# dselivanov/rsparse

Hardware: AMD Instinct MI355X
Metric: als_iterations_per_sec (higher is better)
Workload: dtype f32 (Gram products of rows > 512 / <= 32 non-zeros as 2 x fp16 / 3 x bf16 split terms of the fp32 operands, fp32 accumulate; everything else fp32); 1 GPU; WRMF implicit ALS, CG(3), synthetic 10000000x1000000, 500155883 nnz, rank 128, lambda 0.1; survey_config=3, feedback=implicit, n_items=1000000, nnz=500155883, rank=128, solver=conjugate_gradient, cg_steps=3, parallelism=rows sharded x1, factors replicated

## Files before the change

rsparse_amd/csrc/wrmf_cg_mf.hip:

```cpp
#include <cstdio>
#include <utility>

#pragma clang diagnostic ignored "-Winline-asm"

#include "wrmf_internal.h"
#include "wrmf_device.h"

namespace rsparse_hip {
namespace {
using namespace dev;
constexpr int MF_A0 = 0;
#define MF_TOP "a255"
}
}

#include "wrmf_mf.h"

namespace rsparse_hip {
namespace {

__device__ __forceinline__ void cgm_operands_hi(const float (&x)[16], f16x8& h0, f16x8& h1) {
  float b0[8], b1[8];
#pragma unroll
  for (int e = 0; e < 8; e++) {
// ... 3 lines not shown
  }
  unsigned hh0[4], hh1[4];
#pragma unroll
  for (int q = 0; q < 4; q++) {
    const f32x2 v0 = {b0[2 * q], b0[2 * q + 1]}, v1 = {b1[2 * q], b1[2 * q + 1]};
    hh0[q] = __builtin_bit_cast(unsigned, __builtin_convertvector(v0, f16x2));
    hh1[q] = __builtin_bit_cast(unsigned, __builtin_convertvector(v1, f16x2));
  }
  h0 = pack_f16x8(hh0[0], hh0[1], hh0[2], hh0[3]);
  h1 = pack_f16x8(hh1[0], hh1[1], hh1[2], hh1[3]);
}

struct CgmOps {
  f16x8 ah[4], al[4], mh[4];
};
struct CgmProd {
  int T, kind, K, I;
};
constexpr CgmProd cgm_prod(int idx) {
  if (idx < 16) return {mf_tid(idx % 4, 0), idx / 4, 0, idx % 4};
  idx -= 16;
  if (idx < 12) return {mf_tid(1 + idx % 3, 1), idx / 3, 1, 1 + idx % 3};
  idx -= 12;
  const int w = idx % 3, K = w == 2 ? 3 : 2, I = w == 0 ? 2 : 3;
  return {mf_tid(I, K), idx / 3, K, I};
}
template <int T>
__device__ __forceinline__ void cgm_mma16(const f16x8& a, const f16x8& b) {
  asm volatile("v_mfma_f32_32x32x16_f16 a[%c2:%c3], %0, %1, a[%c2:%c3]" ::"v"(a), "v"(b), "i"(MF_A0 + 16 * T), "i"(MF_A0 + 16 * T + 15));
}

template <int NOPS>
struct CgmWave {
  union {
    float ring[3][2048];
    float T[32 * 36];
  };
  int midx[3][64];
  float mval[3][64];
  float gval[3][64];
  unsigned long long maddr[3][64];
  float vec[128];
  float x0[128];
  float rhs[128];
  double loss;
};
template <int NOPS>
struct CgmSmem {
  float4 G[10][64][4];
  CgmWave<NOPS> w[4];
};

template <class RD, class GV, class WV>
__device__ __forceinline__ void cgm_matvec(RD&& rd, GV&& gtile, WV& sw, const int n, const int hf, const int ln,
                                           const float (&pr)[4], float (&out)[4]) {
  wave_sync();
  if (hf == 0) {
#pragma unroll
    for (int I = 0; I < 4; I++) sw.vec[32 * I + n] = pr[I];
  }
  wave_sync();
  float dsum[4] = {0.f, 0.f, 0.f, 0.f};
  static_for<4>([&](auto kt) {
    constexpr int K = decltype(kt)::value;
    float pc[16];
#pragma unroll
    for (int q = 0; q < 4; q++) {
      const float4 t = *reinterpret_cast<const float4*>(&sw.vec[32 * K + 8 * q + 4 * hf]);
      pc[4 * q] = t.x; pc[4 * q + 1] = t.y; pc[4 * q + 2] = t.z; pc[4 * q + 3] = t.w;
    }
    float ts[16];
#pragma unroll
    for (int v = 0; v < 16; v++) ts[v] = 0.f;
    static_for<4 - K>([&](auto st) {
      constexpr int I = K + decltype(st)::value;
      constexpr int T = mf_tid(I, K);
      float g[16];
      gtile(std::integral_constant<int, T>{}, g);
      static_for<16>([&](auto vt) {
        constexpr int v = decltype(vt)::value;
        const float av = rd(std::integral_constant<int, T>{}, std::integral_constant<int, v>{}) + g[v];
        dsum[I] = fmaf(av, pc[v], dsum[I]);
        if constexpr (I > K) ts[v] = fmaf(av, pr[I], ts[v]);
      });
    });
    if constexpr (K < 3) {
      wave_sync();
#pragma unroll
      for (int v = 0; v < 16; v++) sw.T[(8 * (v >> 2) + 4 * hf + (v & 3)) * 36 + n] = ts[v];
      wave_sync();
      float s0 = 0.f, s1 = 0.f;
#pragma unroll
      for (int q = 0; q < 8; q++) {
        const float4 t = *reinterpret_cast<const float4*>(&sw.T[n * 36 + 4 * q]);
        s0 += t.x + t.z;
        s1 += t.y + t.w;
      }
      out[K] = s0 + s1;
    } else {
      out[K] = 0.f;
    }
  });
#pragma unroll
  for (int I = 0; I < 4; I++) {
    const unsigned du = __float_as_uint(dsum[I]);
    const auto sw2 = __builtin_amdgcn_permlane32_swap(du, du, false, false);
    out[I] += __uint_as_float(sw2[0]) + __uint_as_float(sw2[1]);
  }
}

__device__ __forceinline__ float cgm_dot(const float (&a)[4], const float (&b)[4], const int hf) {
  float s = (a[0] * b[0] + a[1] * b[1]) + (a[2] * b[2] + a[3] * b[3]);
  return wave_sum(hf == 0 ? s : 0.f);
}

template <bool SYM>
__device__ __forceinline__ void als_cg_mf_body(const AlsArgs& a, const int32_t* __restrict__ rows, const int n_rows, const int loss_slot0) {
  extern __shared__ __attribute__((aligned(16))) char cgm_smem[];
  CgmSmem<SYM ? 12 : 20>& sm = *reinterpret_cast<CgmSmem<SYM ? 12 : 20>*>(cgm_smem);
  const int lane = threadIdx.x & 63, wv = rfl((int)(threadIdx.x >> 6));
  CgmWave<SYM ? 12 : 20>& sw = sm.w[wv];
  constexpr int k = 128;
  {
    const bool below_one = a.ne_stats[2] != 0u;
    if (below_one == SYM) {
      if (lane == 0) a.loss_partials[loss_slot0 + 4 * blockIdx.x + wv] = 0.0;
      return;
    }
  }
  for (int e = threadIdx.x; e < 10 * 64 * 16; e += 256) {
    const int t = e / 1024, l = (e >> 4) & 63, v = e & 15;
    const int I = t >= 6 ? 3 : (t >= 3 ? 2 : (t >= 1 ? 1 : 0)), K = t - I * (I + 1) / 2;
    const int nn = l & 31, hh = l >> 5;
    reinterpret_cast<float*>(&sm.G[t][l][0])[v] = a.XtX[(size_t)(4 * (8 * (v >> 2) + 4 * hh + (v & 3)) + K) * k + 4 * nn + I];
  }
  if (lane == 0) sw.loss = 0.0;
  __syncthreads();

  auto uni = [](const float x) { return __int_as_float(__builtin_amdgcn_readfirstlane(__float_as_int(x))); };
  const int ex = rfl(fp16_scale_exp(fmaxf(__uint_as_float(a.ne_stats[0]), 1e-30f)));
  const float wmax = uni(fmaxf(__uint_as_float(a.ne_stats[1]) - 1.f, 1.f));
  const int ewb = rfl((int)((__float_as_uint(wmax) >> 23) & 0xffu));
  const float sx = uni(pow2(ex)), sw_ = uni(pow2(min(253, max(1, 253 - ewb))));
  const float un1 = uni(pow2(254 - ex));
  const float unw = uni(pow2(254 - min(253, max(1, 253 - ewb))));
  const int n_waves = 4 * gridDim.x;

  for (int it = 4 * blockIdx.x + wv; it < n_rows; it += n_waves) {
    const int row = rfl(rows[it]);
    const int p1 = rfl(a.col_ptrs[row]), p2 = rfl(a.col_ptrs[row + 1]);
    float* yrow = a.Y + (size_t)row * k;
    int ln = lane;
    asm volatile("" : "+v"(ln));
    sw.x0[ln] = yrow[ln];
    sw.x0[64 + ln] = yrow[64 + ln];
    MF_DRAIN();
    static_for<256>([&](auto rt) { mf_wr<decltype(rt)::value>(0.f); });
    f32x16 hi[4];
#pragma unroll
    for (int t = 0; t < 4; t++)
#pragma unroll
      for (int e = 0; e < 16; e++) hi[t][e] = 0.f;
    float u0 = 0.f, u1 = 0.f, csum = 0.f;
    float ua[4] = {0.f, 0.f, 0.f, 0.f};
    {
      const int nsteps = (p2 - p1 + 15) >> 4;
      const int hfl = ln >> 5;
      const unsigned long long xoff = reinterpret_cast<unsigned long long>(a.X) + 16ull * (unsigned)(ln & 31);
      const unsigned ring_lds = (unsigned)(uintptr_t)&sw.ring[0][0];
      const unsigned meta_lds = (unsigned)(uintptr_t)&sw.midx[0][0];
      auto request_meta = [&](const int c) __attribute__((always_inline)) {
        const int pos = min(p1 + 64 * c + ln, p2 - 1);
        const int* gi = a.row_idx + pos;
        const float* gv = a.vals + pos;
        const unsigned dst = meta_lds + 256u * (unsigned)(c % 3);
        unsigned keep;
        asm volatile(
            "s_mov_b32 %[k], m0\n\ts_mov_b32 m0, %[l]\n\ts_nop 0\n\t"
            "global_load_lds_dword %[gi], off\n\ts_add_u32 m0, m0, 0x300\n\ts_nop 0\n\t"
            "global_load_lds_dword %[gv], off\n\t"
            "s_mov_b32 m0, %[k]"
            : [k] "=&s"(keep)
            : [l] "s"(dst), [gi] "v"(gi), [gv] "v"(gv)
            : "memory", "scc");
      };
      auto request = [&](const int st, const int slot) __attribute__((always_inline)) {
        const uint4* ap = reinterpret_cast<const uint4*>(&sw.maddr[(st >> 2) % 3][16 * (st & 3) + 8 * hfl]);
        const uint4 q0 = ap[0], q1 = ap[1], q2 = ap[2], q3 = ap[3];
        auto at = [&](const unsigned lo, const unsigned hi2) { return xoff + (((unsigned long long)hi2 << 32) | lo); };
        const unsigned long long g0 = at(q0.x, q0.y), g1 = at(q0.z, q0.w), g2 = at(q1.x, q1.y), g3 = at(q1.z, q1.w);
        const unsigned long long g4 = at(q2.x, q2.y), g5 = at(q2.z, q2.w), g6 = at(q3.x, q3.y), g7 = at(q3.z, q3.w);
        const unsigned dst = ring_lds + 8192u * (unsigned)slot + 4096u;
        unsigned keep;
        asm volatile(
            "s_mov_b32 %[k], m0\n\ts_mov_b32 m0, %[l]\n\ts_nop 0\n\t"
            "global_load_lds_dwordx4 %[g0], off offset:-4096\n\t"
            "global_load_lds_dwordx4 %[g1], off offset:-3072\n\t"
            "global_load_lds_dwordx4 %[g2], off offset:-2048\n\t"
            "global_load_lds_dwordx4 %[g3], off offset:-1024\n\t"
            "global_load_lds_dwordx4 %[g4], off\n\t"
            "global_load_lds_dwordx4 %[g5], off offset:1024\n\t"
            "global_load_lds_dwordx4 %[g6], off offset:2048\n\t"
            "global_load_lds_dwordx4 %[g7], off offset:3072\n\t"
            "s_mov_b32 m0, %[k]"
            : [k] "=&s"(keep)
            : [l] "s"(dst), [g0] "v"(g0), [g1] "v"(g1), [g2] "v"(g2), [g3] "v"(g3), [g4] "v"(g4), [g5] "v"(g5), [g6] "v"(g6), [g7] "v"(g7)
            : "memory");
      };
      auto consume = [&](const int st, const float cvr, float (&xs0)[16], float (&xs1)[16]) __attribute__((always_inline)) {
        const int ccnt = min(16, p2 - (p1 + 16 * st));
        const bool inl = (ln & 15) < ccnt;
        const float cvj = inl ? cvr : 0.f;
        csum += ln < 16 ? cvj : 0.f;
        const float f2 = inl ? sx : 0.f;
        float f1;
        if constexpr (SYM) f1 = inl ? sx * __builtin_amdgcn_sqrtf(fmaxf(cvr - 1.f, 0.f) * sw_) : 0.f;
        else f1 = inl ? (cvr - 1.f) * sw_ : 0.f;
#pragma unroll
        for (int s2 = 0; s2 < 16; s2++) {
          const float cv = readlane_f(cvj, s2);
          u0 = fmaf(cv, xs0[s2], u0);
          u1 = fmaf(cv, xs1[s2], u1);
          const float s_m = readlane_f(f2, s2);
          xs0[s2] *= s_m;
          xs1[s2] *= s_m;
        }
        asm volatile("" : "+v"(u0), "+v"(u1));
        __builtin_amdgcn_sched_barrier(0);
        float (&xm0)[16] = xs0;
        float (&xm1)[16] = xs1;
        f16x8 ah[4], al[4], mh[4], bh[4], bl[4];
        auto m2_products = [&]() __attribute__((always_inline)) {
          static_for<4>([&](auto kt) {
            constexpr int K = decltype(kt)::value;
            static_for<4 - K>([&](auto st2) {
              constexpr int I = K + decltype(st2)::value;
              constexpr int T = mf_tid(I, K);
              if constexpr (T < 6) mf_mma16<10 + T>(mh[K], mh[I]);
// ... 86 lines not shown
        wc[0] = wc0;
        wg[0] = wg0;
        float4 va[2], vb[2];
        va[0] = va0;
        vb[0] = vb0;
        unsigned hm[4][4], hh[4][4], ll[4][4];
        static_for<4>([&](auto qt) {
          constexpr int q = decltype(qt)::value;
          if constexpr (q < 3) {
            va[(q + 1) & 1] = *reinterpret_cast<const float4*>(rs + (2 * q + 2) * 256);
            vb[(q + 1) & 1] = *reinterpret_cast<const float4*>(rs + (2 * q + 3) * 256);
            wc[(q + 1) & 1] = pc[q + 1];
            wg[(q + 1) & 1] = pg[q + 1];
          }
          const float c0 = wc[q & 1].x, c1 = wc[q & 1].y, g0 = wg[q & 1].x, g1 = wg[q & 1].y;
          const float4 xa = va[q & 1], xb = vb[q & 1];
          const float a0s[4] = {xa.x, xa.y, xa.z, xa.w}, a1s[4] = {xb.x, xb.y, xb.z, xb.w};
          static_for<4>([&](auto It) {
            constexpr int I = decltype(It)::value, u = 4 * q + I, m0 = (5 * u) / 2, m1 = (5 * (u + 1)) / 2;
            const float a0 = a0s[I], a1 = a1s[I];
            ua[I] = fmaf(c1, a1, fmaf(c0, a0, ua[I]));
            const float t0 = a0 * sx, t1 = a1 * sx;
            {
              const f32x2 tv = {t0, t1};
              hm[I][q] = __builtin_bit_cast(unsigned, __builtin_convertvector(tv, f16x2));
            }
            mm(std::integral_constant<int, m0>{}, P);
            __builtin_amdgcn_sched_barrier(0);
            {
              const f32x2 yv = {t0 * g0, t1 * g1};
              const unsigned hv = __builtin_bit_cast(unsigned, __builtin_convertvector(yv, f16x2));
              float r0, r1;
              asm("v_fma_mix_f32 %0, %1, %2, -%3 op_sel_hi:[0,0,1]" : "=v"(r0) : "v"(t0), "v"(g0), "v"(hv));
              asm("v_fma_mix_f32 %0, %1, %2, -%3 op_sel:[0,0,1] op_sel_hi:[0,0,1]" : "=v"(r1) : "v"(t1), "v"(g1), "v"(hv));
              const f32x2 rv = {r0, r1};
              hh[I][q] = hv;
              ll[I][q] = __builtin_bit_cast(unsigned, __builtin_convertvector(rv, f16x2));
            }
            mm(std::integral_constant<int, m0 + 1>{}, P);
            if constexpr (m1 - m0 == 3) {
              __builtin_amdgcn_sched_barrier(0);
              mm(std::integral_constant<int, m0 + 2>{}, P);
            }
            __builtin_amdgcn_sched_barrier(0);
          });
        });
#pragma unroll
        for (int I = 0; I < 4; I++) {
          N.mh[I] = pack_f16x8(hm[I][0], hm[I][1], hm[I][2], hm[I][3]);
          N.ah[I] = pack_f16x8(hh[I][0], hh[I][1], hh[I][2], hh[I][3]);
          N.al[I] = pack_f16x8(ll[I][0], ll[I][1], ll[I][2], ll[I][3]);
        }
      };
      wave_sync();
      request_meta(0);
      request_meta(1);
      asm volatile("s_waitcnt vmcnt(0)" ::: "memory");
      transform(0);
      request(0, 0);
      request(1, 1);
      const int tail_st = ((p2 - p1) & 15) ? nsteps - 1 : -1;
      int slot = 0;
      for (int c = 0; 4 * c < nsteps; c++) {
        bool done = false;
        static_for<4>([&](auto jt) {
          constexpr int j = decltype(jt)::value;
          const int st = 4 * c + j;
          if (done || st >= nsteps) { done = true; return; }
          const int slot2 = slot == 0 ? 2 : slot - 1;
          float4 fva, fvb;
          float2 fwc, fwg;
          auto first_reads = [&](const int sl, const int cs, const int jj) __attribute__((always_inline)) {
            const float* rs = &sw.ring[sl][0] + 128 * hfl + 4 * (ln & 31);
            fva = *reinterpret_cast<const float4*>(rs);
            fvb = *reinterpret_cast<const float4*>(rs + 256);
            fwc = *reinterpret_cast<const float2*>(&sw.mval[cs][16 * jj + 8 * hfl]);
            fwg = *reinterpret_cast<const float2*>(&sw.gval[cs][16 * jj + 8 * hfl]);
          };
          if constexpr (j == 1) transform(c + 1);
          const bool more = st + 2 < nsteps;
          if (more) {
            if constexpr (j == 1) asm volatile("s_waitcnt vmcnt(10)" ::: "memory");
            else asm volatile("s_waitcnt vmcnt(8)" ::: "memory");
            if constexpr (SYM) first_reads(slot, c % 3, j);
            request(st + 2, slot2);
            if constexpr (j == 0) request_meta(c + 2);
          } else {
            asm volatile("s_waitcnt vmcnt(0)" ::: "memory");
            if constexpr (SYM) {
              if (st == tail_st) zero_tail(slot, (p2 - p1) & 15);
              first_reads(slot, c % 3, j);
            }
          }
          if constexpr (SYM) {
            __builtin_amdgcn_sched_barrier(0);
            if constexpr (j & 1) step_sym(slot, c % 3, jt, OB, OA, fva, fvb, fwc, fwg);
            else step_sym(slot, c % 3, jt, OA, OB, fva, fvb, fwc, fwg);
          } else {
            const float cvr = sw.mval[c % 3][16 * j + (ln & 15)];
            const float* rs = &sw.ring[slot][0];
            float xs0[16], xs1[16];
#pragma unroll
            for (int s2 = 0; s2 < 16; s2++) {
              xs0[s2] = rs[(s2 & 7) * 256 + (s2 >> 3) * 128 + 4 * (ln & 31) + hfl];
              xs1[s2] = rs[(s2 & 7) * 256 + (s2 >> 3) * 128 + 4 * (ln & 31) + 2 + hfl];
            }
            __builtin_amdgcn_sched_barrier(0);
            consume(st, cvr, xs0, xs1);
            __builtin_amdgcn_sched_barrier(0);
          }
          slot = slot == 2 ? 0 : slot + 1;
        });
        if (done) break;
      }
      if constexpr (SYM) {
        if (nsteps & 1) static_for<40>([&](auto it) { mm(it, OB); });
        else static_for<40>([&](auto it) { mm(it, OA); });
#pragma unroll
        for (int I = 0; I < 4; I++) {
          const unsigned du = __float_as_uint(ua[I]);
          const auto sw2 = __builtin_amdgcn_permlane32_swap(du, du, false, false);
          ua[I] = __uint_as_float(sw2[0]) + __uint_as_float(sw2[1]);
        }
      }
      wave_sync();
    }
    ln = lane;
    asm volatile("" : "+v"(ln));
    const int n = ln & 31, hf = ln >> 5;
    const float un_m1 = (un1 * un1) * (SYM ? unw : unw), un_m2 = un1 * un1;
    MF_DRAIN();
    static_for<160>([&](auto rt) {
      constexpr int R = decltype(rt)::value;
      mf_wr<R>(mf_rd<R>() * un_m1);
    });
    static_for<96>([&](auto rt) {
      constexpr int R = 160 + decltype(rt)::value;
      mf_wr<R>(mf_rd<R>() * un_m2);
    });
    {
      float um = un_m2;
      asm volatile("" : "+v"(um));
#pragma unroll
      for (int t = 0; t < 4; t++)
#pragma unroll
        for (int e = 0; e < 16; e++) hi[t][e] *= um;
    }
    float b[4], x[4];
    if constexpr (SYM) {
#pragma unroll
      for (int I = 0; I < 4; I++) {
        b[I] = ua[I];
        x[I] = sw.x0[4 * n + I];
      }
    } else {
      wave_sync();
      sw.rhs[ln] = u0;
      sw.rhs[64 + ln] = u1;
      wave_sync();
#pragma unroll
      for (int I = 0; I < 4; I++) {
        b[I] = sw.rhs[32 * I + n];
        x[I] = sw.x0[4 * n + I];
      }
    }
    auto rd_m1 = [&](auto tt, auto vt) { return mf_rd<16 * decltype(tt)::value + decltype(vt)::value>(); };
    auto g_tile = [&](auto tt, float (&g)[16]) {
      constexpr int T = decltype(tt)::value;
#pragma unroll
      for (int q = 0; q < 4; q++) {
        const float4 t = sm.G[T][ln][q];
        g[4 * q] = t.x; g[4 * q + 1] = t.y; g[4 * q + 2] = t.z; g[4 * q + 3] = t.w;
      }
    };
    float r[4], p[4], ap[4];
    cgm_matvec(rd_m1, g_tile, sw, n, hf, ln, x, ap);
#pragma unroll
    for (int I = 0; I < 4; I++) { r[I] = b[I] - ap[I]; p[I] = r[I]; }
    double rsold = (double)cgm_dot(r, r, hf);
    for (int stp = 0; stp < a.cg_steps; stp++) {
      cgm_matvec(rd_m1, g_tile, sw, n, hf, ln, p, ap);
      const float alpha = (float)(rsold / (double)cgm_dot(p, ap, hf));
#pragma unroll
      for (int I = 0; I < 4; I++) { x[I] = fmaf(alpha, p[I], x[I]); r[I] = fmaf(-alpha, ap[I], r[I]); }
      const double rsnew = (double)cgm_dot(r, r, hf);
      if (rsnew < (double)kCgTol) break;
      const float beta = (float)(rsnew / rsold);
#pragma unroll
      for (int I = 0; I < 4; I++) p[I] = fmaf(p[I], beta, r[I]);
      rsold = rsnew;
    }
    if (hf == 0) {
      int row2 = row;
      asm volatile("" : "+s"(row2));
      float* yr = a.Y + (size_t)row2 * k;
      *reinterpret_cast<float4*>(yr + 4 * n) = make_float4(x[0], x[1], x[2], x[3]);
    }
    auto rd_m2 = [&](auto tt, auto vt) {
      constexpr int T = decltype(tt)::value, v = decltype(vt)::value;
      if constexpr (T < 6) return mf_rd<160 + 16 * T + v>();
      else return hi[T - 6][v];
    };
    float yMy;
    {
      wave_sync();
      if (hf == 0) {
#pragma unroll
        for (int I = 0; I < 4; I++) sw.vec[32 * I + n] = x[I];
      }
      wave_sync();
      float part = 0.f;
      static_for<4>([&](auto kt) {
        constexpr int K = decltype(kt)::value;
        float pc[16];
#pragma unroll
        for (int q = 0; q < 4; q++) {
          const float4 t = *reinterpret_cast<const float4*>(&sw.vec[32 * K + 8 * q + 4 * hf]);
          pc[4 * q] = t.x; pc[4 * q + 1] = t.y; pc[4 * q + 2] = t.z; pc[4 * q + 3] = t.w;
        }
        static_for<4 - K>([&](auto st) {
          constexpr int I = K + decltype(st)::value;
          constexpr int T = mf_tid(I, K);
          float d = 0.f;
          static_for<16>([&](auto vt) {
            constexpr int v = decltype(vt)::value;
            d = fmaf(rd_m1(std::integral_constant<int, T>{}, vt) + rd_m2(std::integral_constant<int, T>{}, vt), pc[v], d);
          });
          part = fmaf(I == K ? d : 2.f * d, x[I], part);
        });
      });
      yMy = wave_sum(part);
    }
    const float yb = cgm_dot(x, b, hf), yy = cgm_dot(x, x, hf);
    const float sc = wave_sum(csum);
    if (lane == 0) sw.loss += ((double)sc - 2.0 * (double)yb + (double)yMy) + a.lambda_loss * (double)yy;
    wave_sync();
  }
  if (lane == 0) a.loss_partials[loss_slot0 + 4 * blockIdx.x + wv] = sw.loss;
}

}
}

#define CGM_KERNEL(NAME, SYM)                                                                                                     \
  extern "C" __global__ __launch_bounds__(256, 1) __attribute__((amdgpu_num_vgpr(128))) void NAME(                                  \
      rsparse_hip::AlsArgs a, const int32_t* __restrict__ rows, int n_rows, int loss_slot0) {                                       \
    rsparse_hip::als_cg_mf_body<SYM>(a, rows, n_rows, loss_slot0);                                                                  \
  }
CGM_KERNEL(rsparse_hip_als_cg_mf_implicit, true)
CGM_KERNEL(rsparse_hip_als_cg_mf_implicit_any, false)
#undef CGM_KERNEL

namespace rsparse_hip {

bool cg_mf_supported(int k, bool implicit) { return implicit && k == 128; }
int cg_mf_grid(int n_rows) { return std::max(1, std::min((n_rows + 3) / 4, kCgMfGrid)); }
int cg_mf_loss_slots(int n_rows) { return 2 * 4 * cg_mf_grid(n_rows); }

hipError_t launch_als_cg_mf(const AlsArgs& a, const int32_t* rows, int n_rows, int loss_slot0, hipStream_t s, hipEvent_t* ev_slot) {
  if (n_rows <= 0) return hipSuccess;
  if (!a.ne_stats || !cg_mf_supported(a.k, true) || (reinterpret_cast<uintptr_t>(a.X) & 3)) return hipErrorInvalidValue;
  const int grid = cg_mf_grid(n_rows);
  auto kern = rsparse_hip_als_cg_mf_implicit;
  auto kern2 = rsparse_hip_als_cg_mf_implicit_any;
  const int b1 = (int)sizeof(CgmSmem<12>), b2 = (int)sizeof(CgmSmem<20>);
  hipError_t e;
  if ((e = hipFuncSetAttribute(reinterpret_cast<const void*>(kern), hipFuncAttributeMaxDynamicSharedMemorySize, b1)) != hipSuccess) return e;
  if ((e = hipFuncSetAttribute(reinterpret_cast<const void*>(kern2), hipFuncAttributeMaxDynamicSharedMemorySize, b2)) != hipSuccess) return e;
  prof_note(ev_slot, reinterpret_cast<const void*>(kern));
  hipLaunchKernelGGL(kern, dim3(grid), dim3(256), b1, s, a, rows, n_rows, loss_slot0);
  hipLaunchKernelGGL(kern2, dim3(grid), dim3(256), b2, s, a, rows, n_rows, loss_slot0 + 4 * grid);
  return hipGetLastError();
}

}
```

rsparse_amd/build.py:

```python
import subprocess
import sys
import time
from concurrent.futures import ThreadPoolExecutor
from pathlib import Path

PKG = Path(__file__).resolve().parent
CSRC = PKG / "csrc"
SRC = [CSRC / n for n in ("wrmf_kernels.hip", "wrmf_cgq.hip", "wrmf_cgp.hip", "wrmf_ne.hip", "wrmf_chol.hip", "wrmf_chol_wave.hip", "wrmf_chol_mf.hip", "wrmf_cg_mf.hip", "wrmf_chol_lr.hip",
                          "wrmf_topk.hip", "wrmf_topk_large.hip", "wrmf_similar.hip", "wrmf_metrics.hip", "wrmf_hits.hip", "wrmf_lists.hip", "wrmf_diversity.hip", "wrmf_mmr.hip", "wrmf_ranks.hip", "wrmf_score.hip", "wrmf_candidates.hip", "wrmf_sample.hip", "wrmf_sample_weighted.hip", "wrmf_split.hip", "wrmf_confidence.hip", "wrmf_events.hip", "wrmf_explain.hip", "wrmf_init.hip", "wrmf_ingest.hip", "wrmf_nnls.hip", "wrmf_bias.hip", "wrmf_lu.hip",
                          "wrmf_f64.hip", "wrmf_wide.hip", "wrmf_wide_cg.hip", "wrmf_ctx_kernels.hip", "wrmf_schedule.cpp", "wrmf_capi.cpp", "wrmf_f64_capi.cpp", "wrmf_ctx.cpp")]
HEADERS = [CSRC / "wrmf_chol_mf.attrs.csv", CSRC / "wrmf_mf.h", CSRC / "wrmf_internal.h", CSRC / "wrmf_capi_common.h", CSRC / "wrmf_schedule.h", CSRC / "wrmf_device.h", CSRC / "wrmf_sample_team.h", CSRC / "wrmf_wave.h", CSRC / "wrmf_ldlt.h", CSRC / "wrmf_f64.h", PKG.parent / "include" / "rsparse_wrmf_hip.h"]
DEPS = SRC + HEADERS
OUT = PKG / "lib" / "librsparse_wrmf_hip.so"
FLAGS = ["--offload-arch=gfx950", "-O3", "-std=c++17", "-fPIC"]


EXTRA_FLAGS = {n: ["-mllvm", "-forceattrs-csv-path=" + str(CSRC / "wrmf_chol_mf.attrs.csv"), "-fno-slp-vectorize"] for n in ("wrmf_chol_mf.hip", "wrmf_cg_mf.hip")}
AUDITED = {"wrmf_chol_mf.hip", "wrmf_cg_mf.hip"}
REG_LIMIT = {"wrmf_cg_mf.hip": 512}
NO_SPILL = {"wrmf_cgq.hip": ("14als_cgq_kernelILi128ELi24ELi4ELi4E",),
            "wrmf_cgp.hip": ("14als_cgp_kernelILb0ELb1ELi16ELb1E",),
            "wrmf_explain.hip": ("14explain_kernelIfLi128E",),
            "wrmf_sample.hip": ("13sample_kernelILi64E", "13sample_kernelILi256E"),
            "wrmf_sample_weighted.hip": ("22sample_weighted_kernelILi64E", "22sample_weighted_kernelILi256E"),
            "wrmf_hits.hip": ("18hit_metrics_kernelILb0E", "18hit_metrics_kernelILb1E"),
            "wrmf_lists.hip": ("19list_metrics_kernelILb0E", "19list_metrics_kernelILb1E"),
            "wrmf_diversity.hip": ("21list_diversity_kernelI", "21item_inv_norms_kernelI"),
            "wrmf_mmr.hip": ("10mmr_kernelI",),
            "wrmf_confidence.hip": ("conf_moments_kernel", "conf_moments_finish_kernel", "conf_table_kernel", "conf_apply_kernel"),
            "wrmf_events.hip": ("events_pack_kernel", "events_now_kernel", "events_heads_kernel", "events_reduce_kernel",
                                "events_long_chunks_kernel", "events_long_finish_kernel"),
            "wrmf_split.hip": ("split_count_wave_kernel", "split_count_team_kernel", "split_write_wave_kernel", "split_write_team_kernel")}
RESOURCE_FLAG = "-Rpass-analysis=kernel-resource-usage"


def resource_violations(remarks, patterns, limit=256):
    import re
    rows, cur = [], None
    for line in remarks.splitlines():
        m = re.search(r"remark:\s+(.*?) \[-Rpass", line)
        if not m:
            continue
        t = m.group(1).strip()
        if t.startswith("Function Name:"):
            cur = {"name": t.split(":", 1)[1].strip()}
            rows.append(cur)
        elif ":" in t and cur is not None:
            k, v = t.rsplit(":", 1)
            cur[k.strip()] = v.strip()
    bad = []
    for pat in patterns:
        hit = [r for r in rows if pat in r["name"]]
        if not hit:
            bad.append((pat, "no such kernel in the compilation"))
        for r in hit:
            regs = int(r.get("VGPRs", "0")) + int(r.get("AGPRs", "0"))
            for key in ("VGPRs Spill", "ScratchSize [bytes/lane]"):
                if int(r.get(key, "0")):
                    bad.append((r["name"], "%s = %s" % (key, r[key])))
            if regs > limit:
                bad.append((r["name"], "%d vector registers" % regs))
    return bad


def audit_listing(src, extra, obj):
    sys.path.insert(0, str(PKG.parent / "tools" / "dbg"))
    import acc_audit
    lst = obj.with_suffix(".s")

    def listing(flags, floor):
        cmd = ["hipcc", *FLAGS, *flags, "-S", "--cuda-device-only", str(src), "-o", str(lst)]
        r = subprocess.run(cmd, stdout=subprocess.PIPE, stderr=subprocess.PIPE, text=True)
        if r.returncode != 0:
            raise RuntimeError("hipcc -S failed on %s:\n%s" % (src.name, r.stderr[-3000:]))
        acc, flight, _ = acc_audit.audit(str(lst), quiet=True, acc_floor=floor)
        return acc, flight, lst.read_text()
    acc, flight, text = listing(extra, 0)
    import re
    nfree = re.findall(r"\.amdhsa_kernel (\w+)[\s\S]*?\.amdhsa_next_free_vgpr (\d+)", text)
    limit = REG_LIMIT.get(src.name, 256)
    two_waves = bool(nfree) and all(int(v) <= limit for name, v in nfree if "_any" not in name)
    if acc == 0 and flight == 0 and two_waves:
        return
    print("  %s: audit of the two-waves-per-SIMD build failed (accumulator-file %d, in-flight %d, layout ok %s): rebuilding with -DMF_SAFE"
          % (src.name, acc, flight, two_waves), flush=True)
    safe = ["-DMF_SAFE"]
    cmd = ["hipcc", *FLAGS, *safe, "-c", str(src), "-o", str(obj)]
    r = subprocess.run(cmd, stdout=subprocess.PIPE, stderr=subprocess.PIPE, text=True)
    if r.returncode != 0:
        raise RuntimeError("hipcc failed on %s (MF_SAFE):\n%s" % (src.name, r.stderr[-3000:]))
    acc, flight, text = listing(safe, 96)
    if acc or flight:
        raise RuntimeError("%s: the MF_SAFE build fails the audit too (accumulator-file %d, in-flight %d)" % (src.name, acc, flight))


def build(force=False, verbose=False, out=None):
    out = Path(out) if out else OUT
    out.parent.mkdir(exist_ok=True)
    objdir = OUT.parent / "obj"
    objdir.mkdir(parents=True, exist_ok=True)
    src = [s for s in SRC if s.exists()]
    hdr_m = max(h.stat().st_mtime for h in HEADERS)
    todo, objs = [], []
    for s in src:
        o = objdir / (s.stem + ".o")
        objs.append(o)
        if force or not o.exists() or o.stat().st_mtime < max(s.stat().st_mtime, hdr_m):
            todo.append((s, o))
    if not todo and out.exists() and all(out.stat().st_mtime >= o.stat().st_mtime for o in objs):
        return out

    def compile_one(so):
        s, o = so
        t0 = time.time()
        extra = EXTRA_FLAGS.get(s.name, [])
        guard = NO_SPILL.get(s.name)
        cmd = ["hipcc", *FLAGS, *extra, *([RESOURCE_FLAG] if guard else []), "-c", str(s), "-o", str(o)]
        r = subprocess.run(cmd, stdout=subprocess.PIPE, stderr=subprocess.PIPE, text=True)
        if r.returncode != 0:
            raise RuntimeError("hipcc failed on %s:\n%s" % (s.name, r.stderr[-6000:]))
        if guard:
            bad = resource_violations(r.stderr, guard)
            if bad:
                o.unlink()
                raise RuntimeError("%s: kernels that must not spill do:\n%s" % (s.name, "\n".join("  %s: %s" % b for b in bad)))
        if s.name in AUDITED:
            audit_listing(s, extra, o)
        if verbose:
            print("  %-20s %.1f s" % (s.name, time.time() - t0), flush=True)

    with ThreadPoolExecutor(max_workers=8) as ex:
        list(ex.map(compile_one, todo))
    cmd = ["hipcc", "--offload-arch=gfx950", "-fPIC", "-shared", *map(str, objs), "-ldl", "-lpthread", "-o", str(out)]
    subprocess.check_call(cmd)
    return out


if __name__ == "__main__":
    argv = sys.argv[1:]
    outp = argv[argv.index("--out") + 1] if "--out" in argv else None
    t0 = time.time()
    print(build(force="--force" in argv, verbose=True, out=outp), "%.1f s" % (time.time() - t0))
```

rsparse_amd/csrc/wrmf_kernels.hip:

```cpp
#include "wrmf_internal.h"
#include "wrmf_device.h"

namespace rsparse_hip {
namespace {

using namespace dev;

template <int KP, int T, int W, bool IMPLICIT>
struct CgSmem {
  static constexpr int LDT = Geo<KP>::LDT;
  static constexpr size_t gram_floats = IMPLICIT ? (size_t)KP * KP : 0;
  static constexpr size_t tile_floats = (size_t)W * T * LDT;
  static constexpr size_t vec_floats = (size_t)W * KP;
  static constexpr size_t red_floats = (size_t)2 * W * KP + 2 * W;
  static constexpr size_t short_bytes = (gram_floats + tile_floats + vec_floats) * 4 + 16;
  static constexpr size_t long_bytes = (gram_floats + tile_floats + vec_floats + red_floats) * 4 + 16;
};

template <int KP, int W>
__device__ __forceinline__ void load_gram_lds(float* sG, const float* __restrict__ G, int k, int tid) {
  for (int e = tid; e < KP * KP; e += W * 64) {
    const int r = e / KP, c = e % KP;
    sG[e] = (r < k && c < k) ? G[(size_t)r * k + c] : 0.f;
  }
// ... 323 lines not shown
      const int64_t er = ent < n ? ent : n - 1;
#pragma unroll
      for (int mt = 0; mt < NT; mt++) dst[u][mt] = X[er * k + min(mt * 32 + col, k - 1)];
    }
  };
  auto take = [&](const int64_t n0, const float (&src)[U][NT], float (&dst)[U][NT]) {
#pragma unroll
    for (int u = 0; u < U; u++) {
      const bool in = n0 + 2 * u + half < n;
#pragma unroll
      for (int mt = 0; mt < NT; mt++) dst[u][mt] = src[u][mt] * ((in && mt * 32 + col < k) ? 1.f : 0.f);
    }
  };
  float av[U][NT], nx[U][NT];
  const int64_t stride = nw * 2 * U;
  int64_t n0 = gw * 2 * U;
  if (n0 < n) {
    fetch(n0, nx);
    take(n0, nx, av);
  }
  for (; n0 < n; n0 += stride) {
    const bool more = n0 + stride < n;
    if (more) fetch(n0 + stride, nx);
#pragma unroll
    for (int u = 0; u < U; u++)
#pragma unroll
      for (int mt = 0; mt < NT; mt++) amax = fmaxf(amax, fabsf(av[u][mt]));
#pragma unroll
    for (int u = 0; u < U; u++)
#pragma unroll
      for (int mt = 0; mt < NT; mt++)
#pragma unroll
        for (int nt = 0; nt <= mt; nt++)
          acc[mt][nt] = __builtin_amdgcn_mfma_f32_32x32x2f32(av[u][mt], av[u][nt], acc[mt][nt], 0, 0, 0);
    if (more) take(n0 + stride, nx, av);
  }
  if (absmax_bits) {
#pragma unroll
    for (int off = 32; off > 0; off >>= 1) amax = fmaxf(amax, __shfl_xor(amax, off));
    if (lane == 0) atomicMax(absmax_bits, __float_as_uint(amax < 3.0e38f ? amax : 3.0e38f));
  }
  float* out = partials + (size_t)gw * KP * KP;
#pragma unroll
  for (int mt = 0; mt < NT; mt++)
#pragma unroll
    for (int nt = 0; nt <= mt; nt++)
#pragma unroll
      for (int e = 0; e < 16; e++) {
        const int rr = mt * 32 + (e & 3) + 8 * (e >> 2) + 4 * half;
        out[(size_t)rr * KP + nt * 32 + col] = acc[mt][nt][e];
      }
}

__global__ void gramian_reduce_kernel(const float* __restrict__ partials, int nparts, int KP, int k, float ridge,
                                      float* __restrict__ G, double* __restrict__ diag) {
  const int e = blockIdx.x * blockDim.x + threadIdx.x;
  if (e >= k * k) return;
  const int aa = e / k, bb = e % k;
  const int ta = aa / 32, tb = bb / 32;
  const int rr = ta >= tb ? aa : bb, cc = ta >= tb ? bb : aa;
  double s = 0.0;
  const float* src = partials + (size_t)rr * KP + cc;
  for (int w = 0; w < nparts; w++) s += (double)src[(size_t)w * KP * KP];
  G[(size_t)bb * k + aa] = (float)s + (aa == bb ? ridge : 0.f);
  if (aa == bb) diag[aa] = s;
}

__global__ void trace_kernel(const double* __restrict__ diag, int k, double* __restrict__ out) {
  if (threadIdx.x == 0 && blockIdx.x == 0) {
    double s = 0.0;
    for (int i = 0; i < k; i++) s += diag[i];
    *out = s;
  }
}

__global__ __launch_bounds__(256) void weighted_sumsq_kernel(const float* __restrict__ X, int k, int64_t n,
                                                             const float* __restrict__ w, double* __restrict__ partials) {
  __shared__ double sh[4];
  const int64_t total = n * k;
  double s = 0.0;
  for (int64_t e = (int64_t)blockIdx.x * 256 + threadIdx.x; e < total; e += (int64_t)gridDim.x * 256) {
    const float v = X[e];
    const float wj = w ? w[e / k] : 1.f;
    s += (double)(v * v * wj);
  }
  for (int m = 32; m >= 1; m >>= 1) s += __shfl_xor(s, m);
  if ((threadIdx.x & 63) == 0) sh[threadIdx.x >> 6] = s;
  __syncthreads();
  if (threadIdx.x == 0) partials[blockIdx.x] = (sh[0] + sh[1]) + (sh[2] + sh[3]);
}

__global__ __launch_bounds__(256) void sum_partials_kernel(const double* __restrict__ partials, size_t n,
                                                           double* __restrict__ out) {
  __shared__ double sh[4];
  double s = 0.0;
  for (size_t e = threadIdx.x; e < n; e += 256) s += partials[e];
  for (int m = 32; m >= 1; m >>= 1) s += __shfl_xor(s, m);
  if ((threadIdx.x & 63) == 0) sh[threadIdx.x >> 6] = s;
  __syncthreads();
  if (threadIdx.x == 0) *out = (sh[0] + sh[1]) + (sh[2] + sh[3]);
}

__global__ __launch_bounds__(256) void sum_partials_stage_kernel(const double* __restrict__ partials, size_t n,
                                                                 double* __restrict__ tail) {
  __shared__ double sh[4];
  const size_t per = (n + gridDim.x - 1) / gridDim.x, lo = (size_t)blockIdx.x * per, hi = lo + per < n ? lo + per : n;
  double s = 0.0;
  for (size_t e = lo + threadIdx.x; e < hi; e += 256) s += partials[e];
  for (int m = 32; m >= 1; m >>= 1) s += __shfl_xor(s, m);
  if ((threadIdx.x & 63) == 0) sh[threadIdx.x >> 6] = s;
  __syncthreads();
  if (threadIdx.x == 0) tail[blockIdx.x] = (sh[0] + sh[1]) + (sh[2] + sh[3]);
}

__global__ void f64_to_f32_kernel(const double* __restrict__ in, float* __restrict__ out, size_t n) {
  for (size_t e = (size_t)blockIdx.x * blockDim.x + threadIdx.x; e < n; e += (size_t)gridDim.x * blockDim.x)
// ... 65 lines not shown
    if (implicit) return vec ? launch_cg_t<KPV, true, true>(a, s, ev) : launch_cg_t<KPV, true, false>(a, s, ev); \
    return vec ? launch_cg_t<KPV, false, true>(a, s, ev) : launch_cg_t<KPV, false, false>(a, s, ev);             \
  }
  RSP_DISPATCH(32)
  RSP_DISPATCH(64)
  RSP_DISPATCH(128)
#undef RSP_DISPATCH
  return hipErrorInvalidValue;
}

hipError_t launch_sum_partials(const double* partials, size_t n, double* out, hipStream_t s, double* tail) {
  if (tail && n > 16384) {
    hipLaunchKernelGGL(sum_partials_stage_kernel, dim3(kSumStageBlocks), dim3(256), 0, s, partials, n, tail);
    hipError_t err = hipGetLastError();
    if (err != hipSuccess) return err;
    hipLaunchKernelGGL(sum_partials_kernel, dim3(1), dim3(256), 0, s, tail, (size_t)kSumStageBlocks, out);
    return hipGetLastError();
  }
  hipLaunchKernelGGL(sum_partials_kernel, dim3(1), dim3(256), 0, s, partials, n, out);
  return hipGetLastError();
}

static int gramian_waves(int64_t n) {
  int64_t w = (n + 63) / 64;
  if (w < 1) w = 1;
  if (w > 1024) w = 1024;
  return (int)((w + 3) / 4 * 4);
}

size_t gramian_scratch_floats(int k, int64_t n) {
  const int KP = padded_rank(k);
  return (size_t)gramian_waves(n) * KP * KP + 2 * 128  + 16;
}

hipError_t launch_gramian(const float* X, int k, int64_t n, float ridge, float* XtX, double* sumsq,
                          float* scratch, hipStream_t s, hipEvent_t* ev, unsigned* absmax_bits) {
  const int KP = padded_rank(k);
  if (!KP) return hipErrorInvalidValue;
  const int waves = gramian_waves(n);
  float* partials = scratch;
  double* diag = reinterpret_cast<double*>(scratch + (((size_t)waves * KP * KP + 1) & ~(size_t)1));
  const int grid = waves / 4;
  if (ev) (void)hipEventRecord(ev[0], s);
  prof_note(ev, KP == 32 ? reinterpret_cast<const void*>(gramian_partial_kernel<32>)
                         : (KP == 64 ? reinterpret_cast<const void*>(gramian_partial_kernel<64>)
                                     : reinterpret_cast<const void*>(gramian_partial_kernel<128>)));
  prof_note(ev ? ev + 1 : nullptr, reinterpret_cast<const void*>(gramian_reduce_kernel));
  if (KP == 32) hipLaunchKernelGGL(gramian_partial_kernel<32>, dim3(grid), dim3(256), 0, s, X, k, n, partials, absmax_bits);
  else if (KP == 64) hipLaunchKernelGGL(gramian_partial_kernel<64>, dim3(grid), dim3(256), 0, s, X, k, n, partials, absmax_bits);
  else hipLaunchKernelGGL(gramian_partial_kernel<128>, dim3(grid), dim3(256), 0, s, X, k, n, partials, absmax_bits);
  hipError_t err = hipGetLastError();
  if (err != hipSuccess) return err;
  if (ev) (void)hipEventRecord(ev[1], s);
  hipLaunchKernelGGL(gramian_reduce_kernel, dim3((k * k + 255) / 256), dim3(256), 0, s, partials, waves, KP, k,
                     ridge, XtX, diag);
  if ((err = hipGetLastError()) != hipSuccess) return err;
  if (sumsq) {
    hipLaunchKernelGGL(trace_kernel, dim3(1), dim3(64), 0, s, diag, k, sumsq);
    err = hipGetLastError();
  }
  if (ev) (void)hipEventRecord(ev[2], s);
  return err;
}

hipError_t launch_weighted_sumsq(const float* X, int k, int64_t n, const float* w, double* out, double* scratch,
                                 hipStream_t s) {
  int64_t blocks = (n * k + 256 * 16 - 1) / (256 * 16);
  if (blocks < 1) blocks = 1;
  if (blocks > 1024) blocks = 1024;
  hipLaunchKernelGGL(weighted_sumsq_kernel, dim3((int)blocks), dim3(256), 0, s, X, k, n, w, scratch);
  hipError_t err = hipGetLastError();
  if (err != hipSuccess) return err;
  return launch_sum_partials(scratch, (size_t)blocks, out, s);
}

hipError_t launch_f64_to_f32(const double* in, float* out, size_t n, hipStream_t s) {
  if (!n) return hipSuccess;
  size_t blocks = (n + 1023) / 1024;
  if (blocks > 4096) blocks = 4096;
  hipLaunchKernelGGL(f64_to_f32_kernel, dim3((int)blocks), dim3(256), 0, s, in, out, n);
  return hipGetLastError();
}
hipError_t launch_f32_to_f64(const float* in, double* out, size_t n, hipStream_t s) {
  if (!n) return hipSuccess;
  size_t blocks = (n + 1023) / 1024;
  if (blocks > 4096) blocks = 4096;
  hipLaunchKernelGGL(f32_to_f64_kernel, dim3((int)blocks), dim3(256), 0, s, in, out, n);
  return hipGetLastError();
}

}
```

Measured before the change: 8.578 iterations/s.

## Prefetch next row's metadata and initial factors during current row's CG solve

Software-pipelines the per-row loop of the mixed-precision CG kernel. The row index, column pointers, initial Y row and first two metadata chunks for the next row are loaded (via global_load_lds) while the current row's CG iterations run, with row ids and pointers fetched up to three rows ahead. Zeroing of the accumulator registers is moved after the first gather requests are issued. This aims to hide per-row startup latency at the cost of more live scalar state and an added wait/sync before the CG phase. Profiling scripts are also added.

```diff
diff --git a/profiles/cg_mf_row_switch/compare_dumps.py b/profiles/cg_mf_row_switch/compare_dumps.py
--- /dev/null
+++ b/profiles/cg_mf_row_switch/compare_dumps.py
@@ -0,0 +1,13 @@
+import json
+import sys
+from pathlib import Path
+
+import numpy as np
+
+a, b = Path(sys.argv[1]), Path(sys.argv[2])
+out = {}
+for name in ("losses.npy", "user_factors.npy", "item_factors.npy"):
+    x, y = np.load(a / name), np.load(b / name)
+    out[name] = dict(shape=list(x.shape), identical=bool(x.shape == y.shape and x.tobytes() == y.tobytes()))
+print(json.dumps(out))
+sys.exit(0 if all(v["identical"] for v in out.values()) else 1)
diff --git a/profiles/cg_mf_row_switch/dispatches.py b/profiles/cg_mf_row_switch/dispatches.py
--- /dev/null
+++ b/profiles/cg_mf_row_switch/dispatches.py
@@ -0,0 +1,42 @@
+import csv
+import sys
+from pathlib import Path
+
+
+def durations(d):
+    out = {}
+    for f in Path(d).rglob("*kernel_trace.csv"):
+        with open(f) as fh:
+            for r in csv.DictReader(fh):
+                out.setdefault(r["Kernel_Name"], []).append((int(r["End_Timestamp"]) - int(r["Start_Timestamp"])) / 1e6)
+    return out
+
+
+def main():
+    builds = [a.split("=", 1) for a in sys.argv[1:]]
+    tabs = {}
+    for name, d in builds:
+        t = {}
+        for k, v in durations(d).items():
+            if k == "rsparse_hip_als_cg_mf_implicit":
+                cut = (min(v) * max(v)) ** 0.5
+                t[k + " [item side]"] = [x for x in v if x >= cut]
+                t[k + " [user side]"] = [x for x in v if x < cut]
+            else:
+                t[k] = v
+        tabs[name] = t
+    first = tabs[builds[0][0]]
+    keys = sorted(first, key=lambda k: -sum(first[k]))
+    print("%-84s" % "kernel" + "".join("  %-38s" % ("%s: n  mean (min .. max) ms" % n) for n, _ in builds))
+    for k in keys:
+        if sum(first[k]) < 0.5:
+            continue
+        line = "%-84s" % k[:84]
+        for n, _ in builds:
+            v = tabs[n].get(k, [])
+            line += "  %-38s" % ("%3d %8.3f (%.3f .. %.3f)" % (len(v), sum(v) / len(v), min(v), max(v)) if v else "-")
+        print(line)
+
+
+if __name__ == "__main__":
+    main()
diff --git a/profiles/cg_mf_row_switch/measure.py b/profiles/cg_mf_row_switch/measure.py
--- /dev/null
+++ b/profiles/cg_mf_row_switch/measure.py
@@ -0,0 +1,90 @@
+import json
+import os
+import subprocess
+import sys
+from pathlib import Path
+
+ROOT = Path(__file__).resolve().parents[2]
+LENGTHS = (528, 1056, 2112)
+N_ROWS, N_USERS, K, REPS = 65536, 20000, 128, 5
+RESIDENT_WAVES = 1024
+
+
+def child():
+    global N_ROWS
+    if "--rows" in sys.argv:
+        N_ROWS = int(sys.argv[sys.argv.index("--rows") + 1])
+    sys.path.insert(0, str(ROOT))
+    import numpy as np
+    import torch
+    from rsparse_amd.engine import HipBackend
+    be = HipBackend(0)
+    dev = be.device
+    g = torch.Generator(device=dev).manual_seed(7)
+    X = torch.randn(N_USERS, K, generator=g, device=dev) * 0.1
+    G = X.T @ X + 0.1 * torch.eye(K, device=dev)
+    pts = []
+    for L in LENGTHS:
+        p = (torch.arange(N_ROWS + 1, device=dev, dtype=torch.int64) * L).to(torch.int32)
+        i = torch.randint(0, N_USERS, (N_ROWS, L), generator=g, device=dev, dtype=torch.int32).sort(dim=1).values.reshape(-1).contiguous()
+        x = 1.0 + torch.rand(N_ROWS * L, generator=g, device=dev) * 4.0
+        csc = be.make_csc(N_USERS, N_ROWS, p, i, x)
+        info = csc.info()
+        assert info["bucket_rows"][0] == N_ROWS and info["ne_segments"] == 0, info
+        Y0 = torch.randn(N_ROWS, K, generator=g, device=dev) * 0.1
+        loss = torch.zeros(1, dtype=torch.float64, device=dev)
+        ms = []
+        be.profile(True)
+        for rep in range(REPS + 1):
+            Y = Y0.clone()
+            be.half_iteration(csc, True, X, Y, G, 0.1, 1, 3, True, loss)
+            t = be.profile_last()
+            if rep == 0:
+                name = be.profile_last_names()[0]
+                assert "als_cg_mf" in name, name
+            else:
+                ms.append(t[0])
+        be.profile(False)
+        torch.cuda.synchronize()
+        pts.append(dict(L=L, ms=ms, ms_median=float(np.median(ms)), us_per_row=float(np.median(ms)) * 1e3 * RESIDENT_WAVES / N_ROWS,
+                        loss=float(loss.item())))
+        del csc, p, i, x, Y, Y0
+    a, b = np.polyfit([q["L"] for q in pts], [q["us_per_row"] for q in pts], 1)
+    print("RESULT " + json.dumps(dict(a_us_per_nnz=float(a), b_us=float(b), points=pts)), flush=True)
+
+
+def main():
+    argv = sys.argv[1:]
+    if "--child" in argv:
+        return child()
+    libs = [kv.split("=", 1) for kv in argv[argv.index("--libs") + 1].split(",")]
+    rounds = int(argv[argv.index("--rounds") + 1]) if "--rounds" in argv else 3
+    out = Path(argv[argv.index("--out") + 1])
+    res = {name: [] for name, _ in libs}
+    for r in range(rounds):
+        for name, path in libs:
+            env = dict(os.environ, RSPARSE_HIP_LIB=path)
+            pr = subprocess.run(["timeout", "-k", "10", "240", sys.executable, __file__, "--child"] + (["--rows", argv[argv.index("--rows") + 1]] if "--rows" in argv else []), env=env, stdout=subprocess.PIPE,
+                                stderr=subprocess.STDOUT, text=True)
+            line = [l for l in pr.stdout.splitlines() if l.startswith("RESULT ")]
+            if pr.returncode != 0 or not line:
+                print(pr.stdout[-4000:])
+                print("measure: %s failed in round %d with exit status %d: stopping" % (name, r, pr.returncode), flush=True)
+                return 1
+            q = json.loads(line[0][7:])
+            res[name].append(q)
+            print("round %d %-7s a = %.5f us per non-zero   b = %.3f us   (%s)" % (
+                r, name, q["a_us_per_nnz"], q["b_us"], "  ".join("L=%d: %.3f ms" % (p["L"], p["ms_median"]) for p in q["points"])), flush=True)
+    summary = {}
+    for name, qs in res.items():
+        bs = [q["b_us"] for q in qs]
+        summary[name] = dict(b_mean=sum(bs) / len(bs), b_min=min(bs), b_max=max(bs), a_mean=sum(q["a_us_per_nnz"] for q in qs) / len(qs))
+        print("%-7s b = %.3f us (min %.3f, max %.3f, spread %.3f) over %d rounds; a = %.5f" % (
+            name, summary[name]["b_mean"], min(bs), max(bs), max(bs) - min(bs), len(bs), summary[name]["a_mean"]), flush=True)
+    out.parent.mkdir(parents=True, exist_ok=True)
+    out.write_text(json.dumps(dict(summary=summary, runs=res), indent=1))
+    return 0
+
+
+if __name__ == "__main__":
+    sys.exit(main())
diff --git a/rsparse_amd/csrc/wrmf_cg_mf.hip b/rsparse_amd/csrc/wrmf_cg_mf.hip
--- a/rsparse_amd/csrc/wrmf_cg_mf.hip
+++ b/rsparse_amd/csrc/wrmf_cg_mf.hip
@@ -173,21 +173,60 @@
   const float unw = uni(pow2(254 - min(253, max(1, 253 - ewb))));
   const int n_waves = 4 * gridDim.x;
 
-  for (int it = 4 * blockIdx.x + wv; it < n_rows; it += n_waves) {
-    const int row = rfl(rows[it]);
-    const int p1 = rfl(a.col_ptrs[row]), p2 = rfl(a.col_ptrs[row + 1]);
-    float* yrow = a.Y + (size_t)row * k;
+  const unsigned meta_lds = (unsigned)(uintptr_t)&sw.midx[0][0];
+  const unsigned x0_lds = (unsigned)(uintptr_t)&sw.x0[0];
+  auto request_meta_of = [&](const int q1, const int q2, const int c, const int l) __attribute__((always_inline)) {
+    const int pos = min(q1 + 64 * c + l, q2 - 1);
+    const int* gi = a.row_idx + pos;
+    const float* gv = a.vals + pos;
+    const unsigned dst = meta_lds + 256u * (unsigned)(c % 3);
+    unsigned keep;
+    asm volatile(
+        "s_mov_b32 %[k], m0\n\ts_mov_b32 m0, %[l]\n\ts_nop 0\n\t"
+        "global_load_lds_dword %[gi], off\n\ts_add_u32 m0, m0, 0x300\n\ts_nop 0\n\t"
+        "global_load_lds_dword %[gv], off\n\t"
+        "s_mov_b32 m0, %[k]"
+        : [k] "=&s"(keep)
+        : [l] "s"(dst), [gi] "v"(gi), [gv] "v"(gv)
+        : "memory", "scc");
+  };
+  auto request_row = [&](const int rw, const int q1, const int q2) __attribute__((always_inline)) {
+    int l = lane;
+    asm volatile("" : "+v"(l));
+    const float* gy = a.Y + (size_t)rw * k + l;
+    unsigned keep;
+    asm volatile(
+        "s_mov_b32 %[k], m0\n\ts_mov_b32 m0, %[l]\n\ts_nop 0\n\t"
+        "global_load_lds_dword %[gy], off\n\t"
+        "global_load_lds_dword %[gy], off offset:256\n\t"
+        "s_mov_b32 m0, %[k]"
+        : [k] "=&s"(keep)
+        : [l] "s"(x0_lds), [gy] "v"(gy)
+        : "memory");
+    request_meta_of(q1, q2, 0, l);
+    request_meta_of(q1, q2, 1, l);
+  };
+  int it = 4 * blockIdx.x + wv;
+  int row_c = 0, p1_c = 0, p2_c = 0;
+  int row_n = 0, p1_n = 0, p2_n = 0;
+  int row_nn = 0;
+  if (it < n_rows) {
+    row_c = rows[it];
+    if (it + n_waves < n_rows) row_n = rows[it + n_waves];
+    if (it + 2 * n_waves < n_rows) row_nn = rows[it + 2 * n_waves];
+    p1_c = rfl(a.col_ptrs[row_c]);
+    p2_c = rfl(a.col_ptrs[row_c + 1]);
+    if (it + n_waves < n_rows) {
+      p1_n = rfl(a.col_ptrs[row_n]);
+      p2_n = rfl(a.col_ptrs[row_n + 1]);
+    }
+    request_row(row_c, p1_c, p2_c);
+  }
+  for (; it < n_rows; it += n_waves) {
+    const int row = rfl(row_c), p1 = rfl(p1_c), p2 = rfl(p2_c);
     int ln = lane;
     asm volatile("" : "+v"(ln));
-    sw.x0[ln] = yrow[ln];
-    sw.x0[64 + ln] = yrow[64 + ln];
-    MF_DRAIN();
-    static_for<256>([&](auto rt) { mf_wr<decltype(rt)::value>(0.f); });
     f32x16 hi[4];
-#pragma unroll
-    for (int t = 0; t < 4; t++)
-#pragma unroll
-      for (int e = 0; e < 16; e++) hi[t][e] = 0.f;
     float u0 = 0.f, u1 = 0.f, csum = 0.f;
     float ua[4] = {0.f, 0.f, 0.f, 0.f};
     {
@@ -195,22 +234,7 @@
       const int hfl = ln >> 5;
       const unsigned long long xoff = reinterpret_cast<unsigned long long>(a.X) + 16ull * (unsigned)(ln & 31);
       const unsigned ring_lds = (unsigned)(uintptr_t)&sw.ring[0][0];
-      const unsigned meta_lds = (unsigned)(uintptr_t)&sw.midx[0][0];
-      auto request_meta = [&](const int c) __attribute__((always_inline)) {
-        const int pos = min(p1 + 64 * c + ln, p2 - 1);
-        const int* gi = a.row_idx + pos;
-        const float* gv = a.vals + pos;
-        const unsigned dst = meta_lds + 256u * (unsigned)(c % 3);
-        unsigned keep;
-        asm volatile(
-            "s_mov_b32 %[k], m0\n\ts_mov_b32 m0, %[l]\n\ts_nop 0\n\t"
-            "global_load_lds_dword %[gi], off\n\ts_add_u32 m0, m0, 0x300\n\ts_nop 0\n\t"
-            "global_load_lds_dword %[gv], off\n\t"
-            "s_mov_b32 m0, %[k]"
-            : [k] "=&s"(keep)
-            : [l] "s"(dst), [gi] "v"(gi), [gv] "v"(gv)
-            : "memory", "scc");
-      };
+      auto request_meta = [&](const int c) __attribute__((always_inline)) { request_meta_of(p1, p2, c, ln); };
       auto request = [&](const int st, const int slot) __attribute__((always_inline)) {
         const uint4* ap = reinterpret_cast<const uint4*>(&sw.maddr[(st >> 2) % 3][16 * (st & 3) + 8 * hfl]);
         const uint4 q0 = ap[0], q1 = ap[1], q2 = ap[2], q3 = ap[3];
@@ -403,13 +427,16 @@
           N.al[I] = pack_f16x8(ll[I][0], ll[I][1], ll[I][2], ll[I][3]);
         }
       };
-      wave_sync();
-      request_meta(0);
-      request_meta(1);
       asm volatile("s_waitcnt vmcnt(0)" ::: "memory");
       transform(0);
       request(0, 0);
       request(1, 1);
+      MF_DRAIN();
+      static_for<256>([&](auto rt) { mf_wr<decltype(rt)::value>(0.f); });
+#pragma unroll
+      for (int t = 0; t < 4; t++)
+#pragma unroll
+        for (int e = 0; e < 16; e++) hi[t][e] = 0.f;
       const int tail_st = ((p2 - p1) & 15) ? nsteps - 1 : -1;
       int slot = 0;
       for (int c = 0; 4 * c < nsteps; c++) {
@@ -515,6 +542,15 @@
         x[I] = sw.x0[4 * n + I];
       }
     }
+    wave_sync();
+    asm volatile("s_waitcnt lgkmcnt(0)" ::: "memory");
+    if (it + n_waves < n_rows) request_row(row_n, p1_n, p2_n);
+    int q1 = 0, q2 = 0, row_n3 = 0;
+    if (it + 2 * n_waves < n_rows) {
+      q1 = a.col_ptrs[row_nn];
+      q2 = a.col_ptrs[row_nn + 1];
+    }
+    if (it + 3 * n_waves < n_rows) row_n3 = rows[it + 3 * n_waves];
     auto rd_m1 = [&](auto tt, auto vt) { return mf_rd<16 * decltype(tt)::value + decltype(vt)::value>(); };
     auto g_tile = [&](auto tt, float (&g)[16]) {
       constexpr int T = decltype(tt)::value;
@@ -586,6 +622,9 @@
     const float sc = wave_sum(csum);
     if (lane == 0) sw.loss += ((double)sc - 2.0 * (double)yb + (double)yMy) + a.lambda_loss * (double)yy;
     wave_sync();
+    row_c = row_n; p1_c = p1_n; p2_c = p2_n;
+    row_n = row_nn; p1_n = rfl(q1); p2_n = rfl(q2);
+    row_nn = row_n3;
   }
   if (lane == 0) a.loss_partials[loss_slot0 + 4 * blockIdx.x + wv] = sw.loss;
 }
```

Result: no change. 8.595 iterations/s, median of 4 (+0.2%).

## Fold unscale factors into CG matvec and parallelize Gramian partial reduction

Applied to the files above, without the earlier changes.

The CG multi-fragment kernel no longer rescales all 256 accumulator registers and the hi tiles by the unscale factors up front. It applies the factor inside the matvec with an fma, and in the objective term it keeps two separate dot products combined at the end. The Gramian reduce kernel now splits the sum over partials across 16 waves per output element and combines them through shared memory, instead of each thread looping serially over every partial. The build also adds a spill and register-limit guard for the CG kernels. Risks are fp rounding differences and register pressure in the matvec.

```diff
diff --git a/rsparse_amd/build.py b/rsparse_amd/build.py
--- a/rsparse_amd/build.py
+++ b/rsparse_amd/build.py
@@ -30,6 +30,7 @@
             "wrmf_confidence.hip": ("conf_moments_kernel", "conf_moments_finish_kernel", "conf_table_kernel", "conf_apply_kernel"),
             "wrmf_events.hip": ("events_pack_kernel", "events_now_kernel", "events_heads_kernel", "events_reduce_kernel",
                                 "events_long_chunks_kernel", "events_long_finish_kernel"),
+            "wrmf_cg_mf.hip": ("rsparse_hip_als_cg_mf_implicit", "rsparse_hip_als_cg_mf_implicit_any"),
             "wrmf_split.hip": ("split_count_wave_kernel", "split_count_team_kernel", "split_write_wave_kernel", "split_write_team_kernel")}
 RESOURCE_FLAG = "-Rpass-analysis=kernel-resource-usage"
 
@@ -120,7 +121,7 @@
         if r.returncode != 0:
             raise RuntimeError("hipcc failed on %s:\n%s" % (s.name, r.stderr[-6000:]))
         if guard:
-            bad = resource_violations(r.stderr, guard)
+            bad = resource_violations(r.stderr, guard, REG_LIMIT.get(s.name, 256))
             if bad:
                 o.unlink()
                 raise RuntimeError("%s: kernels that must not spill do:\n%s" % (s.name, "\n".join("  %s: %s" % b for b in bad)))
diff --git a/rsparse_amd/csrc/wrmf_cg_mf.hip b/rsparse_amd/csrc/wrmf_cg_mf.hip
--- a/rsparse_amd/csrc/wrmf_cg_mf.hip
+++ b/rsparse_amd/csrc/wrmf_cg_mf.hip
@@ -79,7 +79,7 @@
 };
 
 template <class RD, class GV, class WV>
-__device__ __forceinline__ void cgm_matvec(RD&& rd, GV&& gtile, WV& sw, const int n, const int hf, const int ln,
+__device__ __forceinline__ void cgm_matvec(RD&& rd, GV&& gtile, WV& sw, const float un, const int n, const int hf, const int ln,
                                            const float (&pr)[4], float (&out)[4]) {
   wave_sync();
   if (hf == 0) {
@@ -106,7 +106,7 @@
       gtile(std::integral_constant<int, T>{}, g);
       static_for<16>([&](auto vt) {
         constexpr int v = decltype(vt)::value;
-        const float av = rd(std::integral_constant<int, T>{}, std::integral_constant<int, v>{}) + g[v];
+        const float av = fmaf(rd(std::integral_constant<int, T>{}, std::integral_constant<int, v>{}), un, g[v]);
         dsum[I] = fmaf(av, pc[v], dsum[I]);
         if constexpr (I > K) ts[v] = fmaf(av, pr[I], ts[v]);
       });
@@ -479,24 +479,8 @@
     ln = lane;
     asm volatile("" : "+v"(ln));
     const int n = ln & 31, hf = ln >> 5;
-    const float un_m1 = (un1 * un1) * (SYM ? unw : unw), un_m2 = un1 * un1;
+    const float un_m1 = (un1 * un1) * unw, un_m2 = un1 * un1;
     MF_DRAIN();
-    static_for<160>([&](auto rt) {
-      constexpr int R = decltype(rt)::value;
-      mf_wr<R>(mf_rd<R>() * un_m1);
-    });
-    static_for<96>([&](auto rt) {
-      constexpr int R = 160 + decltype(rt)::value;
-      mf_wr<R>(mf_rd<R>() * un_m2);
-    });
-    {
-      float um = un_m2;
-      asm volatile("" : "+v"(um));
-#pragma unroll
-      for (int t = 0; t < 4; t++)
-#pragma unroll
-        for (int e = 0; e < 16; e++) hi[t][e] *= um;
-    }
     float b[4], x[4];
     if constexpr (SYM) {
 #pragma unroll
@@ -525,12 +509,12 @@
       }
     };
     float r[4], p[4], ap[4];
-    cgm_matvec(rd_m1, g_tile, sw, n, hf, ln, x, ap);
+    cgm_matvec(rd_m1, g_tile, sw, un_m1, n, hf, ln, x, ap);
 #pragma unroll
     for (int I = 0; I < 4; I++) { r[I] = b[I] - ap[I]; p[I] = r[I]; }
     double rsold = (double)cgm_dot(r, r, hf);
     for (int stp = 0; stp < a.cg_steps; stp++) {
-      cgm_matvec(rd_m1, g_tile, sw, n, hf, ln, p, ap);
+      cgm_matvec(rd_m1, g_tile, sw, un_m1, n, hf, ln, p, ap);
       const float alpha = (float)(rsold / (double)cgm_dot(p, ap, hf));
 #pragma unroll
       for (int I = 0; I < 4; I++) { x[I] = fmaf(alpha, p[I], x[I]); r[I] = fmaf(-alpha, ap[I], r[I]); }
@@ -572,11 +556,13 @@
         static_for<4 - K>([&](auto st) {
           constexpr int I = K + decltype(st)::value;
           constexpr int T = mf_tid(I, K);
-          float d = 0.f;
+          float d1 = 0.f, d2 = 0.f;
           static_for<16>([&](auto vt) {
             constexpr int v = decltype(vt)::value;
-            d = fmaf(rd_m1(std::integral_constant<int, T>{}, vt) + rd_m2(std::integral_constant<int, T>{}, vt), pc[v], d);
+            d1 = fmaf(rd_m1(std::integral_constant<int, T>{}, vt), pc[v], d1);
+            d2 = fmaf(rd_m2(std::integral_constant<int, T>{}, vt), pc[v], d2);
           });
+          const float d = fmaf(un_m1, d1, un_m2 * d2);
           part = fmaf(I == K ? d : 2.f * d, x[I], part);
         });
       });
diff --git a/rsparse_amd/csrc/wrmf_kernels.hip b/rsparse_amd/csrc/wrmf_kernels.hip
--- a/rsparse_amd/csrc/wrmf_kernels.hip
+++ b/rsparse_amd/csrc/wrmf_kernels.hip
@@ -399,16 +399,34 @@
       }
 }
 
-__global__ void gramian_reduce_kernel(const float* __restrict__ partials, int nparts, int KP, int k, float ridge,
-                                      float* __restrict__ G, double* __restrict__ diag) {
-  const int e = blockIdx.x * blockDim.x + threadIdx.x;
-  if (e >= k * k) return;
-  const int aa = e / k, bb = e % k;
+constexpr int kGramRedWaves = 16;
+__global__ __launch_bounds__(64 * kGramRedWaves) void gramian_reduce_kernel(const float* __restrict__ partials, int nparts, int KP, int k,
+                                                                            float ridge, float* __restrict__ G, double* __restrict__ diag) {
+  __shared__ double sh[kGramRedWaves][64];
+  const int lane = threadIdx.x & 63, wv = threadIdx.x >> 6;
+  const int e = blockIdx.x * 64 + lane;
+  const bool in = e < k * k;
+  const int ee = in ? e : 0;
+  const int aa = ee / k, bb = ee % k;
   const int ta = aa / 32, tb = bb / 32;
   const int rr = ta >= tb ? aa : bb, cc = ta >= tb ? bb : aa;
+  const int per = (nparts + kGramRedWaves - 1) / kGramRedWaves;
+  const int w0 = min(wv * per, nparts), w1 = min(w0 + per, nparts);
   double s = 0.0;
   const float* src = partials + (size_t)rr * KP + cc;
-  for (int w = 0; w < nparts; w++) s += (double)src[(size_t)w * KP * KP];
+#pragma unroll 8
+  for (int w = w0; w < w1; w++) s += (double)src[(size_t)w * KP * KP];
+  sh[wv][lane] = s;
+  __syncthreads();
+  if (wv != 0 || !in) return;
+  double t[kGramRedWaves];
+#pragma unroll
+  for (int w = 0; w < kGramRedWaves; w++) t[w] = sh[w][lane];
+#pragma unroll
+  for (int m = 1; m < kGramRedWaves; m *= 2)
+#pragma unroll
+    for (int w = 0; w < kGramRedWaves; w += 2 * m) t[w] += t[w + m];
+  s = t[0];
   G[(size_t)bb * k + aa] = (float)s + (aa == bb ? ridge : 0.f);
   if (aa == bb) diag[aa] = s;
 }
@@ -580,7 +598,7 @@
   hipError_t err = hipGetLastError();
   if (err != hipSuccess) return err;
   if (ev) (void)hipEventRecord(ev[1], s);
-  hipLaunchKernelGGL(gramian_reduce_kernel, dim3((k * k + 255) / 256), dim3(256), 0, s, partials, waves, KP, k,
+  hipLaunchKernelGGL(gramian_reduce_kernel, dim3((k * k + 63) / 64), dim3(64 * kGramRedWaves), 0, s, partials, waves, KP, k,
                      ridge, XtX, diag);
   if ((err = hipGetLastError()) != hipSuccess) return err;
   if (sumsq) {
```

Measured after the change: 8.577 iterations/s before, 8.668 iterations/s after (median of 6 runs). 1.01x the previous value.
